# abb128/april-asr

Measured on AMD Instinct MI355X. Metric: audio_seconds_per_second (concurrent 16 kHz sessions x 1/RTF), aprilv0_en-us-sized streaming RNN-T, higher is better.
Workload: dtype f32

## Files before the change

### april_asr_amd/csrc/engine.cc

```cpp
#include "engine.h"
#include <array>
#include <algorithm>
#include <cmath>
#include <chrono>
#include <cstdlib>
#include <cstring>
#include "common.h"
#include "env.h"
#include "rowepi_forms.h"

namespace aprilx {

static size_t align64(size_t x) { return (x + 63) & ~(size_t)63; }

void plan_layout(const NetDims &d, bool has_dec_conv_b, PackedLayout &L)
{
    L.dims = d;
    L.has_dec_conv_b = has_dec_conv_b;
    L.vocab_pad = (d.vocab + 31) & ~31;
    size_t off = 0;
    auto take = [&](size_t n) { size_t o = off; off = align64(off + n); return o; };
    L.k3 = (d.conv_ch[1] * 9 + 63) & ~63;
    L.conv_w[0] = take((size_t)d.conv_ch[0] * 9); L.conv_b[0] = take((size_t)d.conv_ch[0]);
    L.conv_w[1] = take((size_t)d.conv_ch[1] * d.conv_ch[0] * 9); L.conv_b[1] = take((size_t)d.conv_ch[1]);
// ... 363 lines not shown
    for (void *p : {(void *)w_, (void *)wh_, (void *)h_, (void *)c_, (void *)ring_, (void *)eout_, (void *)dout_, (void *)gstate_, (void *)cls_, (void *)ws_, (void *)xin_,
                    (void *)a3_, (void *)de_, (void *)logits_, (void *)rec_d_, (void *)counter_d_,
                    (void *)active_d_, (void *)dirty_d_, (void *)dec_slots_d_,
                    (void *)ds_pcm_[0], (void *)ds_pcm_[1]})
        if (p) (void)hipFree(p);
    for (void *p : {(void *)ring_h_, (void *)step_off_h_, (void *)rec_off_h_, (void *)rec_h_, (void *)logits_h_, (void *)hs_pcm_[0], (void *)hs_pcm_[1]})
        if (p) (void)hipHostFree(p);
    for (int b = 0; b < 2; ++b) if (fb_done_[b]) (void)hipEventDestroy(fb_done_[b]);
    for (int b = 0; b < 2; ++b) if (flight_done_[b]) (void)hipEventDestroy(flight_done_[b]);
    for (void *p : table_allocs_) (void)hipFree(p);
    (void)hipStreamDestroy(stream_); (void)hipStreamDestroy(f_stream_); (void)hipStreamDestroy(s_stream_);
}

void Engine::upload_tables(const FbankHostTables &ft)
{
    auto up = [&](const void *src, size_t bytes) {
        void *p = nullptr;
        HIP_CHECK(hipMalloc(&p, std::max<size_t>(bytes, 16)));
        if (bytes) HIP_CHECK(hipMemcpy(p, src, bytes, hipMemcpyHostToDevice));
        table_allocs_.push_back(p);
        return p;
    };
    ft_.window = (const float *)up(ft.window.data(), ft.window.size() * 4);
    ft_.mel = (const float *)up(ft.mel.data(), ft.mel.size() * 4);
    ft_.mel_lo = (const int *)up(ft.mel_lo.data(), ft.mel_lo.size() * 4);
    ft_.mel_hi = (const int *)up(ft.mel_hi.data(), ft.mel_hi.size() * 4);
    ft_.nfct = (int)ft.factors.size();
    for (int k = 0; k < ft_.nfct; ++k) {
        ft_.fct[k] = ft.factors[(size_t)k];
        ft_.tw[k] = (const double *)up(ft.tw[(size_t)k].data(), ft.tw[(size_t)k].size() * 8);
        ft_.tws[k] = ft.tws[(size_t)k].empty() ? nullptr : (const double *)up(ft.tws[(size_t)k].data(), ft.tws[(size_t)k].size() * 8);
    }
    ft_.padded = ft.padded; ft_.nbins = ft.nbins;
    pad_value_ = ft.pad_value;
}

int Engine::alloc_slot()
{
    std::lock_guard<std::mutex> g(slot_mu_);
    if (free_.empty() && !zero_pending_.empty()) zero_pending_slots();
    if (free_.empty()) return -1;
    const int s = free_.back();
    free_.pop_back();
    ++live_;
    return s;
}

void Engine::zero_pending_slots()
{
    if (zero_pending_.empty()) return;
    if (hipSetDevice(cfg_.device) == hipSuccess) {
        std::lock_guard<std::mutex> cg(capture_mu_);
        m_touched();
        const NetDims &d = L_.dims;
        for (size_t o = 0; o < zero_pending_.size(); o += 64) {
            ZeroSlotArgs z;
            z.h = h_; z.c = c_; z.n_layers = d.n_layers; z.slots = (size_t)cfg_.max_slots; z.d_model = d.d_model; z.hidden = d.hidden;
            z.eout = eout_; z.dout = dout_; z.joiner = d.joiner; z.state = gstate_; z.blank = P_.blank_id; z.h16 = h16_;
            z.n_list = (int)std::min<size_t>(64, zero_pending_.size() - o);
            for (int i = 0; i < z.n_list; ++i) z.list[i] = zero_pending_[o + (size_t)i];
            launch_zero_slot(z, stream_);
        }
    }
    for (int s : zero_pending_) free_.push_back(s);
    zero_pending_.clear();
}
// ... 445 lines not shown
    g.out = xb_ + r0 * d.d_model; g.ldo = d.d_model;
    if (f16_tile_) {
        g.a0 = reinterpret_cast<const float *>(u16_ + r0 * d.hidden); lin16(g, o.whr); g.kz = kzx_hr_;
        g.state16 = h16_ + (size_t)l * S * d.d_model; g.out16 = xb16_ + r0 * d.d_model;
    }
    return g;
}

GemmArgs Engine::args_ff1(int l, size_t r0, int rows) const
{
    const NetDims &d = L_.dims;
    const PackedLayout::Layer &o = L_.layers[(size_t)l];
    GemmArgs g; g.a0 = xb_ + r0 * d.d_model; g.lda0 = d.d_model; g.K0 = d.d_model; lin(g, o.wff1);
    g.M = rows; g.N = d.ffn; g.K = d.d_model; g.kz = 1; g.epi = EPI_BIAS_DSWISH; g.out = ff_ + r0 * d.ffn; g.ldo = d.ffn; g.bias = w_ + o.bff1;
    if (f16_tile_) { g.a0 = reinterpret_cast<const float *>(xb16_ + r0 * d.d_model); lin16(g, o.wff1); g.out = nullptr; g.out16 = ff16_ + r0 * d.ffn; }
    return g;
}

GemmArgs Engine::args_ff2(int l, size_t r0, int rows) const
{
    const NetDims &d = L_.dims;
    const PackedLayout::Layer &o = L_.layers[(size_t)l];
    GemmArgs g; g.a0 = ff_ + r0 * d.ffn; g.lda0 = d.ffn; g.K0 = d.ffn; lin(g, o.wff2);
    g.M = rows; g.N = d.d_model; g.K = d.ffn; g.kz = kz_ff2_; g.tile_ok = tile_ok(); g.force_fullk = 1;
    g.epi = EPI_RESID_SSQ; g.bias = w_ + o.bff2; g.resid = xb_ + r0 * d.d_model; g.ldr = d.d_model; g.out = y_ + r0 * d.d_model; g.ldo = d.d_model; g.ssq_out = ssq_ + r0 * (d.d_model / SSQ_COLS);
    if (f16_tile_) { g.a0 = reinterpret_cast<const float *>(ff16_ + r0 * d.ffn); lin16(g, o.wff2); g.kz = kzx_ff2_; g.out16 = y16_ + r0 * d.d_model; }
    return g;
}

GemmArgs Engine::args_encproj(size_t r0, int rows, const int *slot_idx, float *out) const
{
    const NetDims &d = L_.dims;
    GemmArgs g; g.a0 = y_ + r0 * d.d_model; g.lda0 = d.d_model; g.K0 = d.d_model; lin(g, L_.w_encproj);
    g.M = rows; g.N = d.joiner; g.K = d.d_model; g.kz = kz_proj_; g.tile_ok = tile_ok();
    g.epi = EPI_SLOT_STORE; g.bias = w_ + L_.b_encproj; g.out = out; g.ldo = d.joiner; g.slot_idx = slot_idx; g.x_scale = in_scale(d.n_layers, r0);
    return g;
}


void Engine::launch_rowepi(GemmArgs f, float *ws, hipStream_t st, bool force, int cls)
{
    const int row_cls = cls == T_DEC ? T_DEC : T_ROW;
    f.force_fullk = force ? 1 : 0;
    const GemmPlan p = gemm_plan(f);
    if (p.fused) { timed_begin(cls); launch_gemm(f, st); timed_end(cls); return; }
    timed_begin(cls); launch_gemm(partial_form(f, ws, ws_mstride_), st); timed_end(cls);
    timed_begin(row_cls); launch_row(row_form(f, ws, ws_mstride_, p.planes), st); timed_end(row_cls);
}

void Engine::encoder_front(size_t r0, int rows, const int *row_slots, const float *x_direct, hipStream_t st, float *ws)
{
    const NetDims &d = L_.dims;
    ConvEmbedArgs ca;
    ca.ring = ring_; ca.ring_frames = ring_frames_; ca.mel = d.mel; ca.seg = d.seg;
    ca.slot_idx = row_slots + r0; ca.ring_tail = step_d_ + cfg_.max_batch + r0; ca.x_direct = x_direct;
    for (int i = 0; i < 3; ++i) { ca.w[i] = w_ + L_.conv_w[i]; ca.b[i] = w_ + L_.conv_b[i]; ca.ch[i] = d.conv_ch[i]; ca.stride[i] = d.conv_stride[i]; }
    ca.ch1_per_group = 1;
    for (int k = 8; k > 1; --k) if (d.conv_ch[1] % k == 0) { ca.ch1_per_group = k; break; }
    ca.out = a3_ + r0 * d.f_out * L_.k3; ca.ldo = L_.k3; ca.M = rows;
    if (conv_wt_) { ca.w0t = conv_wt_; ca.w1t = conv_wt_ + (size_t)9 * d.conv_ch[0]; }
    timed_begin(T_CONV); launch_conv_embed(ca, st); timed_end(T_CONV);
    {
        GemmArgs g; g.a0 = ca.out; g.lda0 = L_.k3; g.K0 = L_.k3; g.wp = w_ + L_.conv_w[2];
        g.M = rows * d.f_out; g.N = d.conv_ch[2]; g.K = L_.k3; g.kz = 1; g.epi = EPI_BIAS_DSWISH; g.out = xin_ + r0 * d.embed_in; g.ldo = d.conv_ch[2]; g.bias = w_ + L_.conv_b[2];
        timed_begin(T_CONV); launch_gemm(g, st); timed_end(T_CONV);
    }
    {
        GemmArgs g; g.a0 = xin_ + r0 * d.embed_in; g.lda0 = d.embed_in; g.K0 = d.embed_in; lin(g, L_.w_embed);
        g.M = rows; g.N = d.d_model; g.K = d.embed_in; g.kz = kz_embed_; g.tile_ok = tile_ok();
        g.epi = EPI_RESID_SSQ; g.bias = w_ + L_.b_embed; g.ldr = d.d_model; g.out = y_ + r0 * d.d_model; g.ldo = d.d_model; g.ssq_out = ssq_ + r0 * (d.d_model / SSQ_COLS);
        launch_rowepi(g, ws + r0 * d.d_model, st);
    }
    if (f16_tile_) launch_cvt_f16(y_ + r0 * d.d_model, y16_ + r0 * d.d_model, (size_t)rows * d.d_model, st);
}

void Engine::run_encoder_rows(int n, const float *x_direct)
{
    const NetDims &d = L_.dims;
    encoder_front(0, n, step_d_, x_direct, stream_, ws_);
    for (int l = 0; l < d.n_layers; ++l) {
        timed_begin(T_GATES); launch_gemm(args_gates(l, 0, n, GATES_ALL), stream_); timed_end(T_GATES);
        launch_rowepi(args_whr(l, 0, n), ws_, stream_);
        timed_begin(T_GEMM_OTHER); launch_gemm(args_ff1(l, 0, n), stream_); timed_end(T_GEMM_OTHER);
        launch_rowepi(args_ff2(l, 0, n), ws_, stream_);
    }
    launch_rowepi(args_encproj(0, n, step_d_, eout_), ws_, stream_);
}

DecEmbedParams Engine::dec_params() const
{
    const NetDims &d = L_.dims;
    DecEmbedParams p; p.emb = w_ + L_.emb; p.conv_w = w_ + L_.dec_conv; p.conv_b = L_.has_dec_conv_b ? w_ + L_.dec_conv_b : nullptr;
    p.d = d.d_model; p.groups = d.dec_groups; p.context = d.context; p.vocab = d.vocab;
    return p;
}

void Engine::run_decproj(int n, const int *d_slots, const int *row_mask, const int *run_flag, int run_gen, float *out)
{
    const NetDims &d = L_.dims;
    GemmArgs g; g.a0 = de_; g.lda0 = d.d_model; g.K0 = d.d_model; lin(g, L_.w_decproj);
    g.M = n; g.N = d.joiner; g.K = d.d_model; g.kz = kz_proj_; g.tile_ok = tile_ok(); g.run_flag = run_flag; g.run_gen = run_gen;
    g.epi = EPI_SLOT_STORE; g.bias = w_ + L_.b_decproj; g.out = out ? out : dout_; g.ldo = d.joiner; g.slot_idx = d_slots; g.row_mask = row_mask;
// ... 1228 lines not shown
```

### april_asr_amd/csrc/gemm_debug_api.cc

```cpp
#include <hip/hip_runtime.h>
#include <cstring>
#include <vector>
#include "../../include/aprilx_engine.h"
#include "common.h"
#include "kernels.h"
#include "rowepi_forms.h"

using namespace aprilx;

namespace {

enum { D_N, D_M, D_NC, D_K, D_K0, D_K1, D_KZ, D_EPI, D_AOP, D_WT, D_WAVES, D_TILE_OK, D_FORCE, D_HIDDEN, D_LDO, D_LDA0, D_LDA1, D_LDR, D_LDS, D_LDP,
       D_RUN_FLAG, D_RUN_GEN, D_CTX_VOCAB, D_SAME_B, D_ROWS, D_SLOTS, D_A0_ROWS, D_A1_ROWS, D_A0B_ROWS, D_XG, D_RG, D_OUT, D_OUT16, D_STATE16,
       D_TPIN, D_TPIN_MT, D_TPIN_ZS, D_KPIN, D_KPIN_MT, D_PPIN, D_PPIN_MT };
enum { I_A0, I_A1, I_A0B, I_AIDX0, I_AIDX1, I_AIDX0B, I_SLOT, I_MASK, I_CTX, I_BIAS, I_RESID, I_PADD, I_XSSQ, I_RSSQ, I_CSTATE, I_RESERVED, I_W, N_IN };
enum { O_OUT, O_OUT16, O_STATE, O_STATE16, O_CSTATE, O_SSQ, O_PLANES, N_OUT };
constexpr int MAX_PLANES = 8;

struct Arena {
    std::vector<void *> ptrs;
    bool bad = false;
    bool ok(hipError_t e) { if (e != hipSuccess) { if (!bad) LOGE("aprilx_run_gemm: HIP: %s", hipGetErrorString(e)); bad = true; } return !bad; }
    void *raw(size_t bytes, int fill)
    {
        void *p = nullptr;
        if (bad || !ok(hipMalloc(&p, bytes ? bytes : 4))) return nullptr;
        ptrs.push_back(p);
        ok(hipMemset(p, fill, bytes ? bytes : 4));
        return p;
    }
    void *upload(const void *host, size_t have, size_t bytes)
    {
        void *p = raw(bytes < have ? have : bytes, 0);
        if (p && have) ok(hipMemcpy(p, host, have, hipMemcpyHostToDevice));
        return p;
    }
    void download(void *host, const void *dev, size_t bytes) { if (host && dev && !bad) ok(hipMemcpy(host, dev, bytes, hipMemcpyDeviceToHost)); }
    ~Arena() { for (void *p : ptrs) (void)hipFree(p); }
};

struct Problem {
    GemmArgs g;
    float *planes = nullptr;
    size_t out_rows = 0;
};

}
// ... 2 lines not shown
{
    if (!d || !fd || !in || !out || !plan_out) return -1;
    const int n = d[D_N], M = d[D_M], N = d[D_NC], K = d[D_K];
    const size_t R = (size_t)d[D_ROWS], S = (size_t)d[D_SLOTS];
    if (n < 1 || n > 3 || M < 1 || N < 16 || N % 16 != 0 || K < 64 || K % 64 != 0 || d[D_K0] + d[D_K1] != K) return -1;
    if (R < (size_t)((M + 255) / 256) * 256 || S < 1 || d[D_LDO] < 1 || d[D_LDA0] < d[D_K0] || (d[D_K1] > 0 && d[D_LDA1] < d[D_K1])) return -1;
    const int epi = d[D_EPI];
    const bool row_epi = epi == EPI_HR || epi == EPI_RESID_SSQ || epi == EPI_SLOT_STORE;
    const bool f16 = d[D_WT] == 1, f16_rows = f16 && d[D_TILE_OK] == 2;

    Arena A;
    hipStream_t st = nullptr;
    int *run_flag = nullptr;
    if (d[D_RUN_FLAG] >= 0) { const int v = d[D_RUN_FLAG]; run_flag = (int *)A.upload(&v, sizeof v, sizeof v); }

    auto rows_operand = [&](const void *host, size_t rows, size_t ld) -> const float * {
        if (!host) return nullptr;
        const size_t cnt = (rows < R ? R : rows) * ld;
        float *f = (float *)A.upload(host, rows * ld * 4, cnt * 4);
        if (!f16_rows || !f) return f;
        void *h = A.raw(cnt * 2, 0);
        if (h) launch_cvt_f16(f, h, cnt, st);
        return (const float *)h;
    };
    auto ints = [&](const void *host, size_t have, size_t cnt) -> const int * { return host ? (const int *)A.upload(host, have * 4, cnt * 4) : nullptr; };
    auto floats = [&](const void *host, size_t have, size_t cnt) -> float * { return host ? (float *)A.upload(host, have * 4, cnt * 4) : nullptr; };

    std::vector<Problem> P((size_t)n);
    for (int p = 0; p < n; ++p) {
        const void *const *ip = in + (size_t)p * N_IN;
        GemmArgs &g = P[(size_t)p].g;
        if (!ip[I_A0] || !ip[I_W] || (d[D_K1] > 0 && !ip[I_A1])) return -1;
        g.M = M; g.N = N; g.K = K; g.K0 = d[D_K0]; g.K1 = d[D_K1]; g.kz = d[D_KZ]; g.epi = epi; g.a_op = d[D_AOP]; g.wt = d[D_WT]; g.wave_mask = d[D_WAVES];
        g.tile_ok = d[D_TILE_OK]; g.force_fullk = d[D_FORCE]; g.hidden = d[D_HIDDEN]; g.ldo = d[D_LDO]; g.lda0 = d[D_LDA0]; g.lda1 = d[D_LDA1];
        g.ldr = d[D_LDR]; g.ld_state = d[D_LDS]; g.ldp = d[D_LDP]; g.ctx_vocab = d[D_CTX_VOCAB]; g.same_idx_b = d[D_SAME_B]; g.zcount = n;
        g.run_flag = run_flag; g.run_gen = d[D_RUN_GEN];
        g.a0 = rows_operand(ip[I_A0], (size_t)d[D_A0_ROWS], (size_t)g.lda0);
        g.a1 = rows_operand(ip[I_A1], (size_t)d[D_A1_ROWS], (size_t)g.lda1);
        g.a0b = rows_operand(ip[I_A0B], (size_t)d[D_A0B_ROWS], (size_t)g.lda0);
        g.aidx0 = ints(ip[I_AIDX0], (size_t)M, R); g.aidx1 = ints(ip[I_AIDX1], (size_t)M, R); g.aidx0b = ints(ip[I_AIDX0B], (size_t)M, R);
        g.slot_idx = ints(ip[I_SLOT], (size_t)M, R); g.row_mask = ints(ip[I_MASK], (size_t)M, R);
        g.ctx_state = (const GreedyState *)ints(ip[I_CTX], S * 4, S * 4);
        g.bias = floats(ip[I_BIAS], (size_t)N, (size_t)N);
        g.resid = floats(ip[I_RESID], (size_t)M * g.ldr, R * g.ldr);
        g.p_add = floats(ip[I_PADD], (size_t)M * g.ldp, R * g.ldp);
        if (ip[I_XSSQ]) { g.x_scale.ssq = floats(ip[I_XSSQ], (size_t)M * d[D_XG], R * d[D_XG]); g.x_scale.groups = d[D_XG]; g.x_scale.inv_n = fd[0]; g.x_scale.eps = fd[1]; }
        if (ip[I_RSSQ]) { g.r_scale.ssq = floats(ip[I_RSSQ], (size_t)M * d[D_RG], R * d[D_RG]); g.r_scale.groups = d[D_RG]; g.r_scale.inv_n = fd[2]; g.r_scale.eps = fd[3]; }
        const size_t wn = (size_t)K * N;
        float *w32 = floats(ip[I_W], wn, wn);
        g.wp = w32;
        if (f16 && w32) {
            void *w16 = A.raw(wn * 2, 0);
            if (w16) { if (f16_rows) launch_repack_x32(w32, w16, K, N, st); else launch_cvt_f16(w32, w16, wn, st); }
            g.wp = w16;
        }
        size_t &orows = P[(size_t)p].out_rows;
        orows = (epi == EPI_SLOT_STORE && g.slot_idx) ? S : R;
        if (epi == EPI_PARTIAL) {
            P[(size_t)p].planes = (float *)A.raw((size_t)MAX_PLANES * R * N * 4, 0xFF);
            g.out = P[(size_t)p].planes; g.m_stride = (int)R;
        } else {
            if (d[D_OUT]) g.out = (float *)A.raw(orows * g.ldo * 4, 0xFF);
            if (d[D_OUT16]) g.out16 = A.raw(orows * g.ldo * 2, 0xFF);
            if (epi == EPI_HR) {
                g.state = (float *)A.raw(S * g.ld_state * 4, 0xFF);
                if (d[D_STATE16]) g.state16 = A.raw(S * g.ld_state * 2, 0xFF);
            }
// ... 51 lines not shown
```

### april_asr_amd/csrc/gemm_plan.h

```cpp
#pragma once
#include <algorithm>

namespace aprilx {

enum GemmEpilogue {
    EPI_PARTIAL = 0,
    EPI_LSTM = 1,
    EPI_BIAS_DSWISH = 2,
    EPI_HR = 3,
    EPI_RESID_SSQ = 4,
    EPI_SLOT_STORE = 5,
    EPI_XPART = 6
};
enum GemmAOp { AOP_NONE = 0, AOP_TANH_ADD = 1 };
enum GemmMode { GM_SLAB = 0, GM_FULLK = 1, GM_TILE = 2, GM_KW = 3, GM_PP = 4 };

#define APRIL_KW_TILES(X) X(4, 4) X(2, 2) X(1, 2)
inline bool kw_tile_exists(int mt, int nt)
{
#define X(a, b) if (mt == a && nt == b) return true;
    APRIL_KW_TILES(X)
#undef X
    return false;
}

struct GemmQuery {
    int M = 0, N = 0, K = 0, K0 = 0, K1 = 0, kz = 1;
    int epi = EPI_PARTIAL, a_op = AOP_NONE, wt = 0, wave_mask = 0xF;
    bool has_p_add = false, has_x_scale = false;
    int zcount = 1;
    int tile_ok = 0;
    int force_fullk = 0;
    int recur_form = 0;
    bool kw_ok = false;
    bool pp_ok = false;
    bool pw_ok = false;
};

struct GemmKnobs {
    int fullk = 1;
    int gm_tile = 1;
    int gm_pp = 1;
    int pp_mt = 0;
    int pp_wide = 1;
    int tile_big = 1;
    int tile_f16_fullk = 1;
    int gm_kw = 1;
    int kw_mt = 0;
    int kw_over_tile = 1;
    int z_tiles = 2;
    int tile_enable = -1, tile_pin_mt = 0, tile_pin_zs = 0;
    int pp_enable = -1, pp_pin_mt = 0;
    int kw_enable = -1, kw_pin_mt = 0;
};

enum GemmRoute {
    ROUTE_KSPLIT = 0,
    ROUTE_STREAM = 1,
    ROUTE_PP = 2,
    ROUTE_PW = 3,
    ROUTE_TILE = 4,
    ROUTE_KW = 5
};
enum GemmPlanError {
    PLAN_OK = 0,
    PLAN_ALWAYS_TILE_OPERANDS = 1,
    PLAN_NO_TILE_PLAN = 2,
    PLAN_ROW_NEEDS_FULLK = 3,
    PLAN_XSCALE_SHAPE = 4
};

struct GemmPlan {
    int route = ROUTE_KSPLIT;
    int mode = GM_SLAB, mt = 0, nt = 0, zs = 1;
    int planes = 1;
    bool fused = false;
    int form = 0;
    int error = PLAN_OK;
};

namespace plan_detail {

struct TilePlan { int mt = 0, nt = 0, zs = 1, mode = GM_SLAB; };

struct TileAsk {
    int M, N, kz, zcount;
    bool force_full;
    bool always;
    bool big_ok;
    bool wide_ok;
    bool pp_ok, pw_ok;
};

inline bool is_slab_epi(int epi) { return epi == EPI_LSTM || epi == EPI_BIAS_DSWISH || epi == EPI_XPART; }
inline bool is_row_epi(int epi) { return epi == EPI_HR || epi == EPI_RESID_SSQ || epi == EPI_SLOT_STORE; }

inline bool plan_fullk(int M, int N, int kz, bool force, int zcount, const GemmKnobs &k, TilePlan &t)
{
    constexpr int min_wgs = 96;
    if (!k.fullk || N % 32 != 0) return false;
    const int ncols = N / 32;
    int mt = M <= 16 ? 1 : (M <= 32 ? 2 : 4);
    while (mt > 1 && (long)ncols * ((M + 16 * mt - 1) / (16 * mt)) * zcount < 256) mt >>= 1;
    const long wgs = (long)ncols * ((M + 16 * mt - 1) / (16 * mt)) * zcount;
    if (wgs < min_wgs && !force) return false;
    t.mt = mt; t.nt = 2; t.zs = kz; t.mode = kz >= 4 ? GM_FULLK : GM_SLAB;
    return true;
}

inline bool plan_pp(const TileAsk &a, const GemmKnobs &k, TilePlan &t)
{
    constexpr int min_tiles = 128;
    const int M = a.M, N = a.N;
    if (!(k.pp_enable < 0 ? k.gm_pp : k.pp_enable) || N % 128 != 0) return false;
    const long zc = std::max(1, a.zcount);
    const long t16 = (long)(N / 128) * ((M + 255) / 256) * zc, t8 = (long)(N / 128) * ((M + 127) / 128) * zc;
    int mt = k.pp_pin_mt ? k.pp_pin_mt : k.pp_mt;
    int nt = 8;
    if (mt == 12) { if (!a.pw_ok) return false; mt = 16; nt = 12; }
    else if (mt != 16 && mt != 8) {
        if (t8 < min_tiles) return false;
        const long c16 = ((t16 + 255) / 256) * 100, c8 = ((t8 + 255) / 256) * 60;
        mt = c16 <= c8 ? 16 : 8;
        if (k.pp_wide && a.pw_ok && N % 192 == 0) {
            const long tw = (long)(N / 192) * ((M + 255) / 256) * zc, cw = ((tw + 255) / 256) * 150;
            if (cw < std::min(c16, c8)) { mt = 16; nt = 12; }
        }
    }
    t.mt = mt; t.nt = nt; t.zs = 1; t.mode = GM_PP;
    return true;
}

inline bool plan_tile(const TileAsk &a, const GemmKnobs &k, TilePlan &t)
{
    constexpr int min_rows = 32, fused_tiles = 512, split_tiles = 256;
    const int M = a.M, N = a.N, kz = a.kz;
// ... 16 lines not shown
    else if (pin_zs > 0) { if (!a.force_full) zs = std::min(kz, pin_zs); }
    else if (pin_mt > 0) {  }
    else {
        if (tiles2 < split_tiles && !a.always) return false;
        if (!a.force_full) {
            long best = -1;
            for (int z = kz; z >= 1; z >>= 1) {
                const long wgs = tiles * (kz / z), per_cu = (wgs + 255) / 256;
                long cost = per_cu * (8L * z + 3) * 100;
                if (z < kz) cost += cost / 20 + 300;
                if (best < 0 || cost < best) { best = cost; zs = z; }
            }
        }
    }
    t.mt = mt; t.nt = 4; t.zs = zs; t.mode = GM_TILE;
    return true;
}

inline int plan_tiles(const GemmQuery &q, int epi, bool force_fullk, int tile_ok, int zc_hint, int zc, bool pp_ok, bool pw_ok, const GemmKnobs &k, TilePlan &t)
{
    const int M = q.M, N = q.N, kz = q.kz;
    const bool f16_tile = q.wt == 1 && tile_ok == 2;
    if (tile_ok && (epi == EPI_PARTIAL || is_row_epi(epi) || epi == EPI_LSTM || epi == EPI_BIAS_DSWISH || (epi == EPI_XPART && tile_ok == 2))) {
        TileAsk a;
        a.M = M; a.N = N; a.kz = kz; a.zcount = zc;
        a.force_full = force_fullk || epi != EPI_PARTIAL;
        a.always = tile_ok == 2;
        a.big_ok = f16_tile && is_slab_epi(epi);
        a.wide_ok = tile_ok == 2 && (epi == EPI_PARTIAL || epi == EPI_HR || epi == EPI_RESID_SSQ);
        a.pp_ok = f16_tile && pp_ok; a.pw_ok = a.pp_ok && pw_ok;
        if (plan_tile(a, k, t)) return PLAN_OK;
        if (tile_ok == 2) return PLAN_NO_TILE_PLAN;
    }
    if (!is_slab_epi(epi) && plan_fullk(M, N, kz, force_fullk, zc_hint, k, t)) return PLAN_OK;
    const int ntiles = N / 16;
    t.mode = GM_SLAB;
    t.mt = M <= 16 ? 1 : (M <= 32 ? 2 : 4);
    const int mblocks = (M + t.mt * 16 - 1) / (t.mt * 16);
    t.nt = 4;
    const int z = t.mt == 4 ? zc_hint : 1;
    while (t.nt > 1 && ((ntiles % t.nt) != 0 || (long)(ntiles / t.nt) * mblocks * kz * z < 256)) t.nt >>= 1;
    t.zs = 1;
    if (epi == EPI_PARTIAL) {
        const long tiles = (long)(ntiles / t.nt) * mblocks;
        const int zs_max = (t.mt == 4 && t.nt == 4) ? 4 : 8;
        while (t.zs < kz && t.zs < zs_max && tiles * (kz / (t.zs * 2)) >= 256) t.zs *= 2;
    }
    return PLAN_OK;
}

constexpr int KW_MIN_ROWS = 3;
inline bool kw_enabled(const GemmKnobs &k) { return (k.kw_enable < 0 ? k.gm_kw : k.kw_enable) != 0; }

inline void plan_kw(const GemmQuery &q, int zc, const GemmKnobs &k, TilePlan &t)
{
    if (!kw_enabled(k) || t.zs != q.kz) return;
    if (t.mode == GM_TILE) {
        if (!k.kw_over_tile || t.nt != 4) return;
        const long tiles = (long)(q.N / 64) * ((q.M + 16 * t.mt - 1) / (16 * t.mt)) * zc;
        const long rem = tiles % 512;
        if (!(tiles <= 256 || (tiles > 512 && rem > 0 && rem <= 128))) return;
    }
    if (q.M < KW_MIN_ROWS || (q.epi != EPI_HR && q.epi != EPI_RESID_SSQ)) return;
    if (!q.kw_ok) return;
    int mt = k.kw_pin_mt ? k.kw_pin_mt : k.kw_mt;
    if (!mt) {
        const long t32 = (long)(q.N / 32) * ((q.M + 31) / 32) * zc, t16 = (long)(q.N / 32) * ((q.M + 15) / 16) * zc;
// ... 75 lines not shown
```

### april_asr_amd/csrc/kernels.h

```cpp
#pragma once
#include <hip/hip_runtime.h>
#include <cstdint>
#include "vad.h"
#include "dtmf.h"
#include "tone.h"
#include "gemm_plan.h"

namespace aprilx {



constexpr int SSQ_COLS = 32;

struct RowScale {
    const float *ssq = nullptr;
    int groups = 0;
    float inv_n = 0.0f;
    float eps = 0.0f;
};

struct GreedyState { int32_t ctx0, ctx1; int32_t last_tok; uint32_t last_emit_ms; };

constexpr int STAMP_WORDS = 144, STAMP_ENDS = 8, STAMP_NENDS = 64, STAMP_SUBS = 72;

// ... 2 lines not shown
    const float *a1 = nullptr; int lda1 = 0; const int *aidx1 = nullptr; int K1 = 0;
    const float *a0b = nullptr;
    const int *aidx0b = nullptr; int same_idx_b = 1;
    const GreedyState *ctx_state = nullptr; int ctx_vocab = 0;
    int a_op = AOP_NONE;
    RowScale x_scale;
    const void *wp = nullptr;
    int wt = 0;
    int M = 0, N = 0, K = 0;
    int kz = 1;
    int zs = 1;
    int mode = GM_SLAB;
    int epi = EPI_PARTIAL;
    float *out = nullptr; int ldo = 0;
    void *out16 = nullptr;
    void *state16 = nullptr;
    int m_stride = 0;
    const float *bias = nullptr;
    float *c_state = nullptr;
    const int *slot_idx = nullptr;
    int hidden = 0;
    float *state = nullptr; int ld_state = 0;
    const float *resid = nullptr; int ldr = 0;
    RowScale r_scale;
    float *ssq_out = nullptr;
    const int *row_mask = nullptr;
    const int *run_flag = nullptr;
    int run_gen = 1;
    int wave_mask = 0xF;
    const float *p_add = nullptr; int ldp = 0;
    int force_fullk = 0;
    int zcount = 1;
    int tile_ok = 0;
    int asm_loop = 0;
    unsigned long long *trace = nullptr;
    unsigned long long *stamp = nullptr;
    int debug = 0;
};
void launch_gemm(const GemmArgs &g, hipStream_t s);
void gemm_profile_next_launch(hipEvent_t start, hipEvent_t stop);
bool gemm_profile_pending();
void launch_gemm_tile(const GemmArgs &g, int mt, int nt, const GemmArgs *dev_args, int n, hipStream_t s);
int gemm_kw_waves(const GemmArgs &g);
bool gemm_pp_ok(const GemmArgs &g, int mt);
void launch_gemm_pp(const GemmArgs &g, int mt, const GemmArgs *dev_args, int n, hipStream_t s);
bool gemm_pw_ok(const GemmArgs &g);
void launch_gemm_pw(const GemmArgs &g, const GemmArgs *dev_args, int n, hipStream_t s);
void gemm_pp_pin(int enable, int mt);
void launch_gemm_kw(const GemmArgs &g, int mt, int nt, const GemmArgs *dev_args, int n, hipStream_t s);
void gemm_kw_pin(int enable, int mt);
int recur_form(const GemmArgs &g);
void launch_recur(const GemmArgs &g, int form, const GemmArgs *dev_args, int n, hipStream_t s);
void stage_gemm_z(const GemmArgs *items, int n, GemmArgs *staged);
void launch_gemm_z(const GemmArgs *staged, int n, const GemmArgs *dev_args, hipStream_t s);
GemmPlan gemm_plan(const GemmArgs &g);
GemmQuery gemm_query(const GemmArgs &g);
void gemm_tile_pin(int enable, int mt, int zs);

enum RowMode {
    ROW_HR = 0,
    ROW_RESID_SSQ = 1,
    ROW_SLOT_STORE = 2
};
struct RowArgs {
    int mode = ROW_HR;
    const float *ws = nullptr; int parts = 1; int m_stride = 0; int N = 0; int M = 0;
// ... 154 lines not shown
void launch_block_setup(const BlockSetupArgs &a, hipStream_t s);

struct ConvEmbedArgs {
    const float *ring = nullptr;
    int ring_frames = 0, mel = 0, seg = 0;
    const int *slot_idx = nullptr;
    const int *ring_tail = nullptr;
    const float *w[3] = {nullptr, nullptr, nullptr};
    const float *b[3] = {nullptr, nullptr, nullptr};
    int ch[3] = {0, 0, 0};
    int ch1_per_group = 0;
    int stride[3] = {1, 2, 2};
    float *out = nullptr; int ldo = 0;
    int M = 0;
    const float *x_direct = nullptr;
    const float *w0t = nullptr, *w1t = nullptr;
};
void launch_conv_embed(const ConvEmbedArgs &a, hipStream_t s);
void launch_conv_weight_transpose(const float *w0, const float *w1, int c0, int c1, float *w0t, float *w1t, hipStream_t s);

void launch_cvt_f16(const float *src, void *dst, size_t n, hipStream_t s);

void launch_repack_x32(const float *src_packed, void *dst, int K, int N, hipStream_t s);

struct FbankTables {
    const float *window = nullptr;
    const double *tw[16] = {nullptr};
    const double *tws[16] = {nullptr};
    int fct[16] = {0}; int nfct = 0;
    const float *mel = nullptr;
    const int *mel_lo = nullptr;
    const int *mel_hi = nullptr;
    int padded = 0, nbins = 0;
};
struct FbankFrameDesc { int32_t slot; int32_t ring_row; int32_t pcm_off; };
struct FbankArgs {
    FbankTables t;
    const int16_t *pcm = nullptr;
    const FbankFrameDesc *desc = nullptr;
    int n_frames = 0;
    float *ring = nullptr; int ring_frames = 0;
    float pad_value = 0.0f;
};
void launch_fbank(const FbankArgs &a, hipStream_t s);

struct ResampleDesc {
    const float *taps = nullptr;
    int64_t in_base = 0;
    int64_t out_first = 0;
    int64_t out_end = 0;
    int32_t in_off = 0, in_n = 0;
    int32_t out_dst = 0, out_cnt = 0;
    int32_t L = 1, M = 1, K = 0, ldt = 0;
};
struct ResampleArgs {
    const int16_t *in = nullptr;
    int16_t *out = nullptr;
    const ResampleDesc *desc = nullptr;
    int n_desc = 0;
    int max_blocks = 0;
    int lds_floats = 0;
};
void launch_resample(const ResampleArgs &a, hipStream_t s);

constexpr int kDecodeBlock = 256;
struct DecodeDesc {
    int64_t src_off = 0;
// ... 69 lines not shown
```

### april_asr_amd/csrc/kernels_fbank.hip

```cpp
#include "kernels.h"
#include <atomic>

namespace aprilx {

__device__ __forceinline__ float pcm_to_float(int16_t s) { return (float)s / 32768.0f; }

__device__ void fft_pass4(int ido, int l1, const double *in, double *out, const double *w, int lane)
{
    const double hsqt2 = 0.70710678118654752440;
#define CC(a, b, c) in[(a) + ido * ((b) + l1 * (c))]
#define CH(a, b, c) out[(a) + ido * ((b) + 4 * (c))]
#define WA(x, i) w[(i) + (x) * (ido - 1)]
    for (int k = lane; k < l1; k += 64) {
        const double tr1 = CC(0, k, 3) + CC(0, k, 1);
        CH(0, 2, k) = CC(0, k, 3) - CC(0, k, 1);
        const double tr2 = CC(0, k, 0) + CC(0, k, 2);
        CH(ido - 1, 1, k) = CC(0, k, 0) - CC(0, k, 2);
        CH(0, 0, k) = tr2 + tr1;
        CH(ido - 1, 3, k) = tr2 - tr1;
    }
    if ((ido & 1) == 0) {
        for (int k = lane; k < l1; k += 64) {
            const double ti1 = -hsqt2 * (CC(ido - 1, k, 1) + CC(ido - 1, k, 3));
            const double tr1 = hsqt2 * (CC(ido - 1, k, 1) - CC(ido - 1, k, 3));
            CH(ido - 1, 0, k) = CC(ido - 1, k, 0) + tr1;
            CH(ido - 1, 2, k) = CC(ido - 1, k, 0) - tr1;
            CH(0, 3, k) = ti1 + CC(ido - 1, k, 2);
            CH(0, 1, k) = ti1 - CC(ido - 1, k, 2);
        }
    }
    if (ido > 2) {
        const int nq = (ido - 1) / 2;
        for (int t = lane; t < l1 * nq; t += 64) {
            const int k = t / nq, i = 2 + 2 * (t % nq), ic = ido - i;
            const double cr2 = WA(0, i - 2) * CC(i - 1, k, 1) + WA(0, i - 1) * CC(i, k, 1);
            const double ci2 = WA(0, i - 2) * CC(i, k, 1) - WA(0, i - 1) * CC(i - 1, k, 1);
            const double cr3 = WA(1, i - 2) * CC(i - 1, k, 2) + WA(1, i - 1) * CC(i, k, 2);
            const double ci3 = WA(1, i - 2) * CC(i, k, 2) - WA(1, i - 1) * CC(i - 1, k, 2);
            const double cr4 = WA(2, i - 2) * CC(i - 1, k, 3) + WA(2, i - 1) * CC(i, k, 3);
            const double ci4 = WA(2, i - 2) * CC(i, k, 3) - WA(2, i - 1) * CC(i - 1, k, 3);
            const double tr1 = cr4 + cr2, tr4 = cr4 - cr2;
            const double ti1 = ci2 + ci4, ti4 = ci2 - ci4;
            const double tr2 = CC(i - 1, k, 0) + cr3, tr3 = CC(i - 1, k, 0) - cr3;
            const double ti2 = CC(i, k, 0) + ci3, ti3 = CC(i, k, 0) - ci3;
            CH(i - 1, 0, k) = tr2 + tr1;  CH(ic - 1, 3, k) = tr2 - tr1;
            CH(i, 0, k) = ti1 + ti2;      CH(ic, 3, k) = ti1 - ti2;
            CH(i - 1, 2, k) = tr3 + ti4;  CH(ic - 1, 1, k) = tr3 - ti4;
            CH(i, 2, k) = tr4 + ti3;      CH(ic, 1, k) = tr4 - ti3;
        }
    }
#undef CC
#undef CH
#undef WA
}

__device__ void fft_pass2(int ido, int l1, const double *in, double *out, const double *w, int lane)
{
#define CC(a, b, c) in[(a) + ido * ((b) + l1 * (c))]
#define CH(a, b, c) out[(a) + ido * ((b) + 2 * (c))]
    for (int k = lane; k < l1; k += 64) {
        CH(0, 0, k) = CC(0, k, 0) + CC(0, k, 1);
        CH(ido - 1, 1, k) = CC(0, k, 0) - CC(0, k, 1);
    }
    if ((ido & 1) == 0) {
        for (int k = lane; k < l1; k += 64) {
            CH(0, 1, k) = -CC(ido - 1, k, 1);
            CH(ido - 1, 0, k) = CC(ido - 1, k, 0);
        }
    }
    if (ido > 2) {
        const int nq = (ido - 1) / 2;
        for (int t = lane; t < l1 * nq; t += 64) {
            const int k = t / nq, i = 2 + 2 * (t % nq), ic = ido - i;
            const double tr2 = w[i - 2] * CC(i - 1, k, 1) + w[i - 1] * CC(i, k, 1);
            const double ti2 = w[i - 2] * CC(i, k, 1) - w[i - 1] * CC(i - 1, k, 1);
            CH(i - 1, 0, k) = CC(i - 1, k, 0) + tr2;
            CH(ic - 1, 1, k) = CC(i - 1, k, 0) - tr2;
            CH(i, 0, k) = ti2 + CC(i, k, 0);
            CH(ic, 1, k) = ti2 - CC(i, k, 0);
        }
    }
#undef CC
#undef CH
}

__device__ void fft_pass3(int ido, int l1, const double *in, double *out, const double *w, int lane)
{
    const double taur = -0.5, taui = 0.86602540378443864676;
#define CC(a, b, c) in[(a) + ido * ((b) + l1 * (c))]
#define CH(a, b, c) out[(a) + ido * ((b) + 3 * (c))]
#define WA(x, i) w[(i) + (x) * (ido - 1)]
    for (int k = lane; k < l1; k += 64) {
        const double cr2 = CC(0, k, 1) + CC(0, k, 2);
        CH(0, 0, k) = CC(0, k, 0) + cr2;
        CH(0, 2, k) = taui * (CC(0, k, 2) - CC(0, k, 1));
        CH(ido - 1, 1, k) = CC(0, k, 0) + taur * cr2;
    }
    if (ido > 2) {
        const int nq = (ido - 1) / 2;
        for (int t = lane; t < l1 * nq; t += 64) {
            const int k = t / nq, i = 2 + 2 * (t % nq), ic = ido - i;
            const double dr2 = WA(0, i - 2) * CC(i - 1, k, 1) + WA(0, i - 1) * CC(i, k, 1);
            const double di2 = WA(0, i - 2) * CC(i, k, 1) - WA(0, i - 1) * CC(i - 1, k, 1);
            const double dr3 = WA(1, i - 2) * CC(i - 1, k, 2) + WA(1, i - 1) * CC(i, k, 2);
            const double di3 = WA(1, i - 2) * CC(i, k, 2) - WA(1, i - 1) * CC(i - 1, k, 2);
            const double cr2 = dr2 + dr3, ci2 = di2 + di3;
            CH(i - 1, 0, k) = CC(i - 1, k, 0) + cr2;
            CH(i, 0, k) = CC(i, k, 0) + ci2;
            const double tr2 = CC(i - 1, k, 0) + taur * cr2;
            const double ti2 = CC(i, k, 0) + taur * ci2;
            const double tr3 = taui * (di2 - di3);
            const double ti3 = taui * (dr3 - dr2);
            CH(i - 1, 2, k) = tr2 + tr3;  CH(ic - 1, 1, k) = tr2 - tr3;
            CH(i, 2, k) = ti3 + ti2;      CH(ic, 1, k) = ti3 - ti2;
        }
    }
#undef CC
// ... 103 lines not shown
            re += cs[2 * a1] * X2(ik, j) + cs[2 * a2] * X2(ik, j + 1);
            im += cs[2 * a1 + 1] * X2(ik, jc) + cs[2 * a2 + 1] * X2(ik, jc - 1);
        }
        for (; j < half; ++j, --jc) {
            ang += l; if (ang >= ip) ang -= ip;
            re += cs[2 * ang] * X2(ik, j);
            im += cs[2 * ang + 1] * X2(ik, jc);
        }
        Y2(ik, l) = re;
        Y2(ik, ip - l) = im;
    }
    __syncthreads();
    for (int t = lane; t < l1 * ido; t += 64) { const int i = t % ido, k = t / ido; XO(i, 0, k) = Y1(i, k, 0); }
    for (int t = lane; t < (half - 1) * l1 * (nq + 1); t += 64) {
        const int q = t % (nq + 1), k = (t / (nq + 1)) % l1, j = 1 + t / ((nq + 1) * l1), jc = ip - j, j2 = 2 * j - 1;
        if (q == nq) {
            XO(ido - 1, j2, k) = Y1(0, k, j);
            XO(0, j2 + 1, k) = Y1(0, k, jc);
        } else {
            const int i = 1 + 2 * q, ic = ido - i - 2;
            XO(i, j2 + 1, k) = Y1(i, k, j) + Y1(i, k, jc);
            XO(ic, j2, k) = Y1(i, k, j) - Y1(i, k, jc);
            XO(i + 1, j2 + 1, k) = Y1(i + 1, k, j) + Y1(i + 1, k, jc);
            XO(ic + 1, j2, k) = Y1(i + 1, k, jc) - Y1(i + 1, k, j);
        }
    }
#undef X1
#undef X2
#undef Y2
#undef Y1
#undef XO
}

__global__ __launch_bounds__(64) void fbank_kernel(FbankArgs a)
{
    extern __shared__ __attribute__((aligned(16))) double sh[];
    const int lane = threadIdx.x;
    const FbankFrameDesc d = a.desc[blockIdx.x];
    const int n = a.t.padded, nbins = a.t.nbins, nfft = n >> 1;
    float *out = a.ring + ((size_t)d.slot * a.ring_frames + d.ring_row) * nbins;
    if (d.pcm_off < 0) {
        for (int m = lane; m < nbins; m += 64) out[m] = a.pad_value;
        return;
    }
    const int16_t *pcm = a.pcm + d.pcm_off;
    double *A = sh, *B = sh + n;

    float mean;
    if (n <= 512) {
        int part = 0;
        for (int j = lane; j < n; j += 64) part += (int)pcm[j];
#pragma unroll
        for (int off = 32; off > 0; off >>= 1) part += __shfl_xor(part, off);
        const float sum = (float)part / 32768.0f;
        mean = sum / (float)n;
    } else {
        float sum = 0.0f;
        if (lane == 0) for (int j = 0; j < n; ++j) sum = (float)((double)sum + (double)pcm_to_float(pcm[j]));
        sum = __shfl(sum, 0);
        mean = sum / (float)n;
    }
    const double pe = (double)0.97f;
    for (int j = lane; j < n; j += 64) {
        const double dj = (double)pcm_to_float(pcm[j]) - (double)mean;
        const double dp = j > 0 ? (double)pcm_to_float(pcm[j - 1]) - (double)mean : dj;
        double v = dj - pe * dp;
        v *= (double)a.t.window[j];
        A[j] = v;
    }
    __syncthreads();

    double *src = A, *dst = B;
    int l1 = n;
    for (int k1 = 0; k1 < a.t.nfct; ++k1) {
        const int k = a.t.nfct - k1 - 1;
        const int ip = a.t.fct[k];
        const int ido = n / l1;
        l1 /= ip;
        if (ip == 4) fft_pass4(ido, l1, src, dst, a.t.tw[k], lane);
        else if (ip == 2) fft_pass2(ido, l1, src, dst, a.t.tw[k], lane);
        else if (ip == 3) fft_pass3(ido, l1, src, dst, a.t.tw[k], lane);
        else if (ip == 5) fft_pass5(ido, l1, src, dst, a.t.tw[k], lane);
        else { fft_pass_generic(ido, ip, l1, src, dst, a.t.tw[k], a.t.tws[k], lane); __syncthreads(); continue; }
        __syncthreads();
        double *t = src; src = dst; dst = t;
    }
    float *pw = reinterpret_cast<float *>(dst);
    for (int k = lane; k < nfft; k += 64) {
        const float re = (float)(k == 0 ? src[0] : src[2 * k - 1]);
        const float im = (float)(k == 0 ? 0.0 : src[2 * k]);
        pw[k] = re * re + im * im;
    }
    __syncthreads();
    const float kFloor = 1.1920928955078125e-07f;
    for (int m = lane; m < nbins; m += 64) {
        const float *w = a.t.mel + (size_t)m * nfft;
        float val = 0.0f;
        const int hi = a.t.mel_hi[m];
        for (int k0 = a.t.mel_lo[m]; k0 < hi; k0 += 8) {
            float wv[8], pv[8];
#pragma unroll
            for (int i = 0; i < 8; ++i) { const int k = k0 + i < hi ? k0 + i : hi - 1; wv[i] = w[k]; pv[i] = pw[k]; }
#pragma unroll
            for (int i = 0; i < 8; ++i) if (k0 + i < hi) val += pv[i] * wv[i];
        }
        const float v = kFloor > val ? kFloor : val;
        out[m] = (float)log((double)v);
    }
}

void launch_fbank(const FbankArgs &a, hipStream_t s)
{
    if (a.n_frames <= 0) return;
    const size_t lds = sizeof(double) * 2 * (size_t)a.t.padded;
    if (lds > 64 * 1024) {
        static std::atomic<uint64_t> attr_devs{0};
        int dev = 0;
        (void)hipGetDevice(&dev);
        const uint64_t bit = 1ull << (dev & 63);
        if (!(attr_devs.load(std::memory_order_acquire) & bit)) {
            (void)hipFuncSetAttribute(reinterpret_cast<const void *>(&fbank_kernel), hipFuncAttributeMaxDynamicSharedMemorySize, 160 * 1024);
            attr_devs.fetch_or(bit, std::memory_order_release);
        }
    }
    hipLaunchKernelGGL(fbank_kernel, dim3((unsigned)a.n_frames), dim3(64), lds, s, a);
}

}
```

### april_asr_amd/csrc/kernels_gemm.hip

```cpp
#include "kernels.h"
#include "../../include/aprilx_engine.h"
#include "device_utils.h"
#include "env.h"
#ifndef APRIL_ASM_LOOP_ALIGN
#define APRIL_ASM_LOOP_ALIGN ".p2align 3\n"
#endif
#include "gemm_mainloop_asm.inc"
#ifndef APRIL_ASM_NB
#define APRIL_ASM_NB 2
#endif
#include <algorithm>
#include <cstdlib>

namespace aprilx {


template <int MT, int NT>
struct TileCfg {
    static constexpr int BM = MT * 16, BN = NT * 16, LDR = BN + 4;
    static constexpr int LDS_FLOATS = 4 * BM * LDR;
};

template <int WT> struct WQuad { using type = f32x4; };
template <> struct WQuad<1> { using type = h4; };
// ... 579 lines not shown
    if constexpr (EPI == EPI_LSTM) stamp_end(stamp, gridDim.x, blockIdx.x);
}

template <int EPI, int AOP, int MODE>
__global__ __launch_bounds__(256, 1) void gemm_f32_zkernel_mixed(const GemmArgs *__restrict__ zargs, int gx4, int gy, int nbig_problems)
{
    const int nbig = gx4 * gy * nbig_problems;
    int tile = (int)blockIdx.x;
    if (tile < nbig) {
        const int bx = tile % gx4, r = tile / gx4, by = r % gy, z = r / gy;
        const GemmArgs g = zargs[z];
        gemm_body<4, 4, EPI, AOP, 0, MODE, 1>(g, 0, (unsigned)tile, bx, by, gy == 1);
    } else {
        tile -= nbig;
        const int gx2 = 2 * gx4, bx = tile % gx2, by = tile / gx2;
        const GemmArgs g = zargs[nbig_problems];
        gemm_body<4, 2, EPI, AOP, 0, MODE, 1>(g, 0, (unsigned)(nbig + tile), bx, by, gy == 1);
    }
}

ProfileEvents &tl_profile_events() { static thread_local ProfileEvents pe; return pe; }
void gemm_profile_next_launch(hipEvent_t start, hipEvent_t stop) { ProfileEvents &pe = tl_profile_events(); pe.a = start; pe.b = stop; }
bool gemm_profile_pending() { return tl_profile_events().a != nullptr; }

static GemmKnobs &knobs()
{
    static GemmKnobs k = [] {
        GemmKnobs e;
        e.fullk = env_int("APRIL_FULLK", 1); e.gm_tile = env_int("APRIL_GM_TILE", 1);
        e.gm_pp = env_int("APRIL_GM_PP", 1); e.pp_mt = env_int("APRIL_PP_MT", 0); e.pp_wide = env_int("APRIL_PP_WIDE", 1);
        e.tile_big = env_int("APRIL_TILE_BIG", 1); e.tile_f16_fullk = env_int("APRIL_TILE_F16_FULLK", 1);
        e.gm_kw = env_int("APRIL_GM_KW", 1); e.kw_mt = env_int("APRIL_KW_MT", 0); e.kw_over_tile = env_int("APRIL_KW_OVER_TILE", 1);
        e.z_tiles = env_int("APRIL_Z_TILES", 2);
        return e;
    }();
    return k;
}
void gemm_tile_pin(int enable, int mt, int zs) { GemmKnobs &k = knobs(); k.tile_enable = enable; k.tile_pin_mt = mt; k.tile_pin_zs = zs; }
void gemm_pp_pin(int enable, int mt) { GemmKnobs &k = knobs(); k.pp_enable = enable; k.pp_pin_mt = mt; }
void gemm_kw_pin(int enable, int mt) { GemmKnobs &k = knobs(); k.kw_enable = enable; k.kw_pin_mt = mt; }

GemmQuery gemm_query(const GemmArgs &g)
{
    GemmQuery q;
    q.M = g.M; q.N = g.N; q.K = g.K; q.K0 = g.K0; q.K1 = g.K1; q.kz = g.kz; q.epi = g.epi; q.a_op = g.a_op; q.wt = g.wt; q.wave_mask = g.wave_mask;
    q.has_p_add = g.p_add != nullptr; q.has_x_scale = g.x_scale.ssq != nullptr;
    q.zcount = g.zcount; q.tile_ok = g.tile_ok; q.force_fullk = g.force_fullk;
    q.recur_form = recur_form(g); q.kw_ok = gemm_kw_waves(g) != 0; q.pp_ok = gemm_pp_ok(g, 16); q.pw_ok = gemm_pw_ok(g);
    return q;
}
GemmPlan gemm_plan(const GemmArgs &g) { return plan_gemm(gemm_query(g), knobs()); }

[[noreturn]] static void plan_die(const GemmArgs &g, int error)
{
    switch (error) {
    case PLAN_ALWAYS_TILE_OPERANDS: fprintf(stderr, "libapril(mi355x): launch_gemm: always-tile GEMM with a prologue / wave mask / odd N\n"); break;
    case PLAN_NO_TILE_PLAN: fprintf(stderr, "libapril(mi355x): launch_gemm: no GM_TILE plan for an always-tile GEMM (M=%d N=%d kz=%d)\n", g.M, g.N, g.kz); break;
    case PLAN_ROW_NEEDS_FULLK: fprintf(stderr, "libapril(mi355x): launch_gemm: row epilogue %d needs the full-K plan (M=%d N=%d kz=%d)\n", g.epi, g.M, g.N, g.kz); break;
    default: fprintf(stderr, "libapril(mi355x): launch_gemm: x_scale needs K0 == K / 2 and kz == 1\n"); break;
    }
    abort();
}

static void finalize_gemm(GemmArgs &g, const GemmPlan &p)
{
    static const int dbg = env_int("APRIL_GEMM_DEBUG", 0);
    static const int asm_loop = env_int("APRIL_GEMM_ASM", 1);
    if (p.error) plan_die(g, p.error);
    g.zs = p.zs; g.mode = p.mode; g.debug = dbg;
    g.asm_loop = asm_loop != 0;
}

template <int MT, int NT, int EPI, int AOP, int MODE, bool Z>
static void launch_one(const GemmArgs &g, const GemmArgs *dev_args, int n, hipStream_t s)
{
    constexpr bool HAS_ASM = MODE == GM_SLAB && MT == 4 && (NT == 4 || NT == 2) && AOP == AOP_NONE && (EPI == EPI_LSTM || EPI == EPI_BIAS_DSWISH);
    using Cfg = TileCfg<MT, NT>;
    const int zdiv = MODE == GM_FULLK ? 1 : g.kz / g.zs;
    dim3 grid((unsigned)(g.N / Cfg::BN), (unsigned)((g.M + Cfg::BM - 1) / Cfg::BM), (unsigned)(zdiv * (dev_args ? n : 1)));
    const size_t lds = (Cfg::LDS_FLOATS + scale_lds_floats(g, Cfg::BM)) * sizeof(float);
// ... 130 lines not shown
```

Measured before the change: 20070.

## Specialize 512-point fbank FFT on LDS and use taller tiles for lone GEMMs

Adds a templated fbank kernel for the common 512-point FFT plan (factors 2,4,4,4,4). It fixes the pass sequence at compile time and uses explicit LDS address-space pointers, so loop dispatch and generic address handling are avoided. Separately, the embed and encoder-projection GEMMs are flagged as standalone tall GEMMs, and the full-K planner then picks 64-row tiles when the 32-row tile count lands between 256 and 512 workgroups. Both changes can be switched off through environment knobs. Larger tiles halve the workgroup count and may lower occupancy.

```diff
diff --git a/april_asr_amd/csrc/engine.cc b/april_asr_amd/csrc/engine.cc
--- a/april_asr_amd/csrc/engine.cc
+++ b/april_asr_amd/csrc/engine.cc
@@ -419,6 +419,7 @@
         ft_.tws[k] = ft.tws[(size_t)k].empty() ? nullptr : (const double *)up(ft.tws[(size_t)k].data(), ft.tws[(size_t)k].size() * 8);
     }
     ft_.padded = ft.padded; ft_.nbins = ft.nbins;
+    ft_.plan512 = (fbank_plan_is_512(ft_) && env_int("APRIL_FBANK_512", 1) != 0) ? 1 : 0;
     pad_value_ = ft.pad_value;
 }
 
@@ -930,7 +931,7 @@
 {
     const NetDims &d = L_.dims;
     GemmArgs g; g.a0 = y_ + r0 * d.d_model; g.lda0 = d.d_model; g.K0 = d.d_model; lin(g, L_.w_encproj);
-    g.M = rows; g.N = d.joiner; g.K = d.d_model; g.kz = kz_proj_; g.tile_ok = tile_ok();
+    g.M = rows; g.N = d.joiner; g.K = d.d_model; g.kz = kz_proj_; g.tile_ok = tile_ok(); g.lone_tall = 1;
     g.epi = EPI_SLOT_STORE; g.bias = w_ + L_.b_encproj; g.out = out; g.ldo = d.joiner; g.slot_idx = slot_idx; g.x_scale = in_scale(d.n_layers, r0);
     return g;
 }
@@ -965,7 +966,7 @@
     }
     {
         GemmArgs g; g.a0 = xin_ + r0 * d.embed_in; g.lda0 = d.embed_in; g.K0 = d.embed_in; lin(g, L_.w_embed);
-        g.M = rows; g.N = d.d_model; g.K = d.embed_in; g.kz = kz_embed_; g.tile_ok = tile_ok();
+        g.M = rows; g.N = d.d_model; g.K = d.embed_in; g.kz = kz_embed_; g.tile_ok = tile_ok(); g.lone_tall = 1;
         g.epi = EPI_RESID_SSQ; g.bias = w_ + L_.b_embed; g.ldr = d.d_model; g.out = y_ + r0 * d.d_model; g.ldo = d.d_model; g.ssq_out = ssq_ + r0 * (d.d_model / SSQ_COLS);
         launch_rowepi(g, ws + r0 * d.d_model, st);
     }
diff --git a/april_asr_amd/csrc/gemm_debug_api.cc b/april_asr_amd/csrc/gemm_debug_api.cc
--- a/april_asr_amd/csrc/gemm_debug_api.cc
+++ b/april_asr_amd/csrc/gemm_debug_api.cc
@@ -12,7 +12,7 @@
 
 enum { D_N, D_M, D_NC, D_K, D_K0, D_K1, D_KZ, D_EPI, D_AOP, D_WT, D_WAVES, D_TILE_OK, D_FORCE, D_HIDDEN, D_LDO, D_LDA0, D_LDA1, D_LDR, D_LDS, D_LDP,
        D_RUN_FLAG, D_RUN_GEN, D_CTX_VOCAB, D_SAME_B, D_ROWS, D_SLOTS, D_A0_ROWS, D_A1_ROWS, D_A0B_ROWS, D_XG, D_RG, D_OUT, D_OUT16, D_STATE16,
-       D_TPIN, D_TPIN_MT, D_TPIN_ZS, D_KPIN, D_KPIN_MT, D_PPIN, D_PPIN_MT };
+       D_TPIN, D_TPIN_MT, D_TPIN_ZS, D_KPIN, D_KPIN_MT, D_PPIN, D_PPIN_MT, D_LONE_TALL };
 enum { I_A0, I_A1, I_A0B, I_AIDX0, I_AIDX1, I_AIDX0B, I_SLOT, I_MASK, I_CTX, I_BIAS, I_RESID, I_PADD, I_XSSQ, I_RSSQ, I_CSTATE, I_RESERVED, I_W, N_IN };
 enum { O_OUT, O_OUT16, O_STATE, O_STATE16, O_CSTATE, O_SSQ, O_PLANES, N_OUT };
 constexpr int MAX_PLANES = 8;
@@ -81,7 +81,7 @@
         GemmArgs &g = P[(size_t)p].g;
         if (!ip[I_A0] || !ip[I_W] || (d[D_K1] > 0 && !ip[I_A1])) return -1;
         g.M = M; g.N = N; g.K = K; g.K0 = d[D_K0]; g.K1 = d[D_K1]; g.kz = d[D_KZ]; g.epi = epi; g.a_op = d[D_AOP]; g.wt = d[D_WT]; g.wave_mask = d[D_WAVES];
-        g.tile_ok = d[D_TILE_OK]; g.force_fullk = d[D_FORCE]; g.hidden = d[D_HIDDEN]; g.ldo = d[D_LDO]; g.lda0 = d[D_LDA0]; g.lda1 = d[D_LDA1];
+        g.tile_ok = d[D_TILE_OK]; g.force_fullk = d[D_FORCE]; g.lone_tall = d[D_LONE_TALL]; g.hidden = d[D_HIDDEN]; g.ldo = d[D_LDO]; g.lda0 = d[D_LDA0]; g.lda1 = d[D_LDA1];
         g.ldr = d[D_LDR]; g.ld_state = d[D_LDS]; g.ldp = d[D_LDP]; g.ctx_vocab = d[D_CTX_VOCAB]; g.same_idx_b = d[D_SAME_B]; g.zcount = n;
         g.run_flag = run_flag; g.run_gen = d[D_RUN_GEN];
         g.a0 = rows_operand(ip[I_A0], (size_t)d[D_A0_ROWS], (size_t)g.lda0);
diff --git a/april_asr_amd/csrc/gemm_plan.h b/april_asr_amd/csrc/gemm_plan.h
--- a/april_asr_amd/csrc/gemm_plan.h
+++ b/april_asr_amd/csrc/gemm_plan.h
@@ -31,6 +31,7 @@
     int zcount = 1;
     int tile_ok = 0;
     int force_fullk = 0;
+    bool lone_tall = false;
     int recur_form = 0;
     bool kw_ok = false;
     bool pp_ok = false;
@@ -48,6 +49,7 @@
     int gm_kw = 1;
     int kw_mt = 0;
     int kw_over_tile = 1;
+    int fullk_tall = 1;
     int z_tiles = 2;
     int tile_enable = -1, tile_pin_mt = 0, tile_pin_zs = 0;
     int pp_enable = -1, pp_pin_mt = 0;
@@ -95,13 +97,17 @@
 inline bool is_slab_epi(int epi) { return epi == EPI_LSTM || epi == EPI_BIAS_DSWISH || epi == EPI_XPART; }
 inline bool is_row_epi(int epi) { return epi == EPI_HR || epi == EPI_RESID_SSQ || epi == EPI_SLOT_STORE; }
 
-inline bool plan_fullk(int M, int N, int kz, bool force, int zcount, const GemmKnobs &k, TilePlan &t)
+inline bool plan_fullk(int M, int N, int kz, bool force, int zcount, const GemmKnobs &k, TilePlan &t, bool alone = false)
 {
     constexpr int min_wgs = 96;
     if (!k.fullk || N % 32 != 0) return false;
     const int ncols = N / 32;
     int mt = M <= 16 ? 1 : (M <= 32 ? 2 : 4);
     while (mt > 1 && (long)ncols * ((M + 16 * mt - 1) / (16 * mt)) * zcount < 256) mt >>= 1;
+    if (alone && k.fullk_tall && mt == 2 && kz >= 4) {
+        const long wgs2 = (long)ncols * ((M + 31) / 32);
+        if (wgs2 > 256 && wgs2 < 512) mt = 4;
+    }
     const long wgs = (long)ncols * ((M + 16 * mt - 1) / (16 * mt)) * zcount;
     if (wgs < min_wgs && !force) return false;
     t.mt = mt; t.nt = 2; t.zs = kz; t.mode = kz >= 4 ? GM_FULLK : GM_SLAB;
@@ -184,7 +190,7 @@
         if (plan_tile(a, k, t)) return PLAN_OK;
         if (tile_ok == 2) return PLAN_NO_TILE_PLAN;
     }
-    if (!is_slab_epi(epi) && plan_fullk(M, N, kz, force_fullk, zc_hint, k, t)) return PLAN_OK;
+    if (!is_slab_epi(epi) && plan_fullk(M, N, kz, force_fullk, zc_hint, k, t, zc == 1 && q.lone_tall)) return PLAN_OK;
     const int ntiles = N / 16;
     t.mode = GM_SLAB;
     t.mt = M <= 16 ? 1 : (M <= 32 ? 2 : 4);
diff --git a/april_asr_amd/csrc/kernels.h b/april_asr_amd/csrc/kernels.h
--- a/april_asr_amd/csrc/kernels.h
+++ b/april_asr_amd/csrc/kernels.h
@@ -58,6 +58,7 @@
     int force_fullk = 0;
     int zcount = 1;
     int tile_ok = 0;
+    int lone_tall = 0;
     int asm_loop = 0;
     unsigned long long *trace = nullptr;
     unsigned long long *stamp = nullptr;
@@ -278,7 +279,9 @@
     const int *mel_lo = nullptr;
     const int *mel_hi = nullptr;
     int padded = 0, nbins = 0;
-};
+    int plan512 = 0;
+};
+bool fbank_plan_is_512(const FbankTables &t);
 struct FbankFrameDesc { int32_t slot; int32_t ring_row; int32_t pcm_off; };
 struct FbankArgs {
     FbankTables t;
diff --git a/april_asr_amd/csrc/kernels_fbank.hip b/april_asr_amd/csrc/kernels_fbank.hip
--- a/april_asr_amd/csrc/kernels_fbank.hip
+++ b/april_asr_amd/csrc/kernels_fbank.hip
@@ -1,11 +1,16 @@
 #include "kernels.h"
 #include <atomic>
+#include <type_traits>
 
 namespace aprilx {
 
 __device__ __forceinline__ float pcm_to_float(int16_t s) { return (float)s / 32768.0f; }
 
-__device__ void fft_pass4(int ido, int l1, const double *in, double *out, const double *w, int lane)
+using lds_double = __attribute__((address_space(3))) double;
+using lds_float = __attribute__((address_space(3))) float;
+
+template <class P>
+__device__ __forceinline__ void pass4_body(const int ido, const int l1, const P in, const P out, const double *w, const int lane)
 {
     const double hsqt2 = 0.70710678118654752440;
 #define CC(a, b, c) in[(a) + ido * ((b) + l1 * (c))]
@@ -53,8 +58,10 @@
 #undef CH
 #undef WA
 }
-
-__device__ void fft_pass2(int ido, int l1, const double *in, double *out, const double *w, int lane)
+__device__ void fft_pass4(int ido, int l1, double *in, double *out, const double *w, int lane) { pass4_body<double *>(ido, l1, in, out, w, lane); }
+
+template <class P>
+__device__ __forceinline__ void pass2_body(const int ido, const int l1, const P in, const P out, const double *w, const int lane)
 {
 #define CC(a, b, c) in[(a) + ido * ((b) + l1 * (c))]
 #define CH(a, b, c) out[(a) + ido * ((b) + 2 * (c))]
@@ -83,6 +90,7 @@
 #undef CC
 #undef CH
 }
+__device__ void fft_pass2(int ido, int l1, double *in, double *out, const double *w, int lane) { pass2_body<double *>(ido, l1, in, out, w, lane); }
 
 __device__ void fft_pass3(int ido, int l1, const double *in, double *out, const double *w, int lane)
 {
@@ -252,19 +260,22 @@
 #undef XO
 }
 
-__global__ __launch_bounds__(64) void fbank_kernel(FbankArgs a)
+template <bool PLAN512>
+__device__ __forceinline__ void fbank_frame(const FbankArgs &a)
 {
     extern __shared__ __attribute__((aligned(16))) double sh[];
+    using DP = typename std::conditional<PLAN512, lds_double *, double *>::type;
+    using FP = typename std::conditional<PLAN512, lds_float *, float *>::type;
     const int lane = threadIdx.x;
     const FbankFrameDesc d = a.desc[blockIdx.x];
-    const int n = a.t.padded, nbins = a.t.nbins, nfft = n >> 1;
+    const int n = PLAN512 ? 512 : a.t.padded, nbins = a.t.nbins, nfft = n >> 1;
     float *out = a.ring + ((size_t)d.slot * a.ring_frames + d.ring_row) * nbins;
     if (d.pcm_off < 0) {
         for (int m = lane; m < nbins; m += 64) out[m] = a.pad_value;
         return;
     }
     const int16_t *pcm = a.pcm + d.pcm_off;
-    double *A = sh, *B = sh + n;
+    const DP A = (DP)sh, B = A + n;
 
     float mean;
     if (n <= 512) {
@@ -290,7 +301,15 @@
     }
     __syncthreads();
 
-    double *src = A, *dst = B;
+    DP src = A, dst = B;
+    if constexpr (PLAN512) {
+        pass4_body<DP>(1, 128, A, B, a.t.tw[4], lane); __syncthreads();
+        pass4_body<DP>(4, 32, B, A, a.t.tw[3], lane); __syncthreads();
+        pass4_body<DP>(16, 8, A, B, a.t.tw[2], lane); __syncthreads();
+        pass4_body<DP>(64, 2, B, A, a.t.tw[1], lane); __syncthreads();
+        pass2_body<DP>(256, 1, A, B, a.t.tw[0], lane); __syncthreads();
+        src = B; dst = A;
+    } else {
     int l1 = n;
     for (int k1 = 0; k1 < a.t.nfct; ++k1) {
         const int k = a.t.nfct - k1 - 1;
@@ -305,7 +324,8 @@
         __syncthreads();
         double *t = src; src = dst; dst = t;
     }
-    float *pw = reinterpret_cast<float *>(dst);
+    }
+    const FP pw = (FP)dst;
     for (int k = lane; k < nfft; k += 64) {
         const float re = (float)(k == 0 ? src[0] : src[2 * k - 1]);
         const float im = (float)(k == 0 ? 0.0 : src[2 * k]);
@@ -329,6 +349,14 @@
     }
 }
 
+__global__ __launch_bounds__(64) void fbank_kernel(FbankArgs a) { fbank_frame<false>(a); }
+__global__ __launch_bounds__(64) void fbank512_kernel(FbankArgs a) { fbank_frame<true>(a); }
+
+bool fbank_plan_is_512(const FbankTables &t)
+{
+    return t.padded == 512 && t.nfct == 5 && t.fct[0] == 2 && t.fct[1] == 4 && t.fct[2] == 4 && t.fct[3] == 4 && t.fct[4] == 4;
+}
+
 void launch_fbank(const FbankArgs &a, hipStream_t s)
 {
     if (a.n_frames <= 0) return;
@@ -343,7 +371,8 @@
             attr_devs.fetch_or(bit, std::memory_order_release);
         }
     }
-    hipLaunchKernelGGL(fbank_kernel, dim3((unsigned)a.n_frames), dim3(64), lds, s, a);
-}
-
-}
+    if (a.t.plan512) hipLaunchKernelGGL(fbank512_kernel, dim3((unsigned)a.n_frames), dim3(64), lds, s, a);
+    else hipLaunchKernelGGL(fbank_kernel, dim3((unsigned)a.n_frames), dim3(64), lds, s, a);
+}
+
+}
diff --git a/april_asr_amd/csrc/kernels_gemm.hip b/april_asr_amd/csrc/kernels_gemm.hip
--- a/april_asr_amd/csrc/kernels_gemm.hip
+++ b/april_asr_amd/csrc/kernels_gemm.hip
@@ -635,6 +635,7 @@
         e.tile_big = env_int("APRIL_TILE_BIG", 1); e.tile_f16_fullk = env_int("APRIL_TILE_F16_FULLK", 1);
         e.gm_kw = env_int("APRIL_GM_KW", 1); e.kw_mt = env_int("APRIL_KW_MT", 0); e.kw_over_tile = env_int("APRIL_KW_OVER_TILE", 1);
         e.z_tiles = env_int("APRIL_Z_TILES", 2);
+        e.fullk_tall = env_int("APRIL_FULLK_TALL", 1);
         return e;
     }();
     return k;
@@ -648,7 +649,7 @@
     GemmQuery q;
     q.M = g.M; q.N = g.N; q.K = g.K; q.K0 = g.K0; q.K1 = g.K1; q.kz = g.kz; q.epi = g.epi; q.a_op = g.a_op; q.wt = g.wt; q.wave_mask = g.wave_mask;
     q.has_p_add = g.p_add != nullptr; q.has_x_scale = g.x_scale.ssq != nullptr;
-    q.zcount = g.zcount; q.tile_ok = g.tile_ok; q.force_fullk = g.force_fullk;
+    q.zcount = g.zcount; q.tile_ok = g.tile_ok; q.force_fullk = g.force_fullk; q.lone_tall = g.lone_tall != 0;
     q.recur_form = recur_form(g); q.kw_ok = gemm_kw_waves(g) != 0; q.pp_ok = gemm_pp_ok(g, 16); q.pw_ok = gemm_pw_ok(g);
     return q;
 }
```

New measurement: 20070, median of 2. About the same (-0.0%).
